# Niema-Lab/AmpliPy

Hardware: AMD Instinct MI355X
Metric: aligned reads/s through trim+pileup+call, 30 kb ref @ 10k x depth (higher is better)
Workload: dtype u8/int32

## Files before the change

### amplipy_amd/build.py

```python
from __future__ import annotations

import os
import shutil
import subprocess

_HERE = os.path.dirname(os.path.abspath(__file__))
CSRC = os.path.join(_HERE, "csrc")
UNITS = ["amplihip.hip", "amp_readpass.hip", "amp_ins.hip", "amp_deflate.hip", "amp_sam.hip", "amp_bgzf.hip", "amp_qc.hip", "amp_strand.hip", "amp_amplicon.hip",
         "amp_codon.hip", "amp_del.hip", "amp_insev.hip", "amp_cooc.hip", "amp_errprof.hip", "amp_hap.hip", "amp_readpos.hip"]
HEADERS = [os.path.join(_HERE, "..", "include", "amplihip.h")] + sorted(os.path.join(CSRC, f) for f in os.listdir(CSRC) if f.endswith(".hpp"))
UNIT_DEPS = {"amplihip.hip": [os.path.join(_HERE, "..", "include", "amplihip.h")] + [os.path.join(CSRC, f) for f in
                              ("amp_ctx.hpp", "amp_read.hpp", "amp_plan.hpp", "amp_hook.hpp", "amp_call.hpp", "amp_ins.hpp", "amp_codec.hpp")],
             "amp_readpass.hip": [os.path.join(_HERE, "..", "include", "amplihip.h")] + [os.path.join(CSRC, f) for f in
                                  ("amp_ctx.hpp", "amp_read.hpp", "amp_plan.hpp", "amp_hook.hpp", "amp_tile.hpp", "amp_bf.hpp", "amp_fast.hpp",
                                   "amp_fast5.hpp", "amp_fast6.hpp", "amp_fast7.hpp", "amp_wave.hpp", "amp_heavy.hpp")],
             "amp_ins.hip": [os.path.join(_HERE, "..", "include", "amplihip.h"), os.path.join(CSRC, "amp_ins.hpp")],
             "amp_deflate.hip": [os.path.join(_HERE, "..", "include", "amplihip.h")],
             "amp_qc.hip": [os.path.join(_HERE, "..", "include", "amplihip.h")] + [os.path.join(CSRC, f) for f in ("amp_hook.hpp", "amp_qc.hpp", "amp_clip.hpp", "amp_strand.hpp", "amp_tally.hpp")],
             "amp_strand.hip": [os.path.join(_HERE, "..", "include", "amplihip.h")] + [os.path.join(CSRC, f) for f in ("amp_hook.hpp", "amp_strand.hpp", "amp_tally.hpp")],
             "amp_amplicon.hip": [os.path.join(_HERE, "..", "include", "amplihip.h")] + [os.path.join(CSRC, f) for f in ("amp_hook.hpp", "amp_strand.hpp", "amp_amplicon.hpp", "amp_tally.hpp")],
             "amp_codon.hip": [os.path.join(_HERE, "..", "include", "amplihip.h")] + [os.path.join(CSRC, f) for f in ("amp_hook.hpp", "amp_strand.hpp", "amp_codon.hpp", "amp_tally.hpp")],
             "amp_del.hip": [os.path.join(_HERE, "..", "include", "amplihip.h")] + [os.path.join(CSRC, f) for f in ("amp_hook.hpp", "amp_strand.hpp", "amp_del.hpp", "amp_keyed.hpp", "amp_tally.hpp")],
             "amp_insev.hip": [os.path.join(_HERE, "..", "include", "amplihip.h")] + [os.path.join(CSRC, f) for f in ("amp_hook.hpp", "amp_strand.hpp", "amp_insev.hpp", "amp_keyed.hpp", "amp_ins.hpp", "amp_readpos.hpp", "amp_tally.hpp")],
             "amp_cooc.hip": [os.path.join(_HERE, "..", "include", "amplihip.h")] + [os.path.join(CSRC, f) for f in ("amp_hook.hpp", "amp_strand.hpp", "amp_cooc.hpp", "amp_tally.hpp")],
             "amp_errprof.hip": [os.path.join(_HERE, "..", "include", "amplihip.h")] + [os.path.join(CSRC, f) for f in ("amp_hook.hpp", "amp_strand.hpp", "amp_errprof.hpp", "amp_tally.hpp")],
             "amp_hap.hip": [os.path.join(_HERE, "..", "include", "amplihip.h")] + [os.path.join(CSRC, f) for f in ("amp_hook.hpp", "amp_strand.hpp", "amp_hap.hpp", "amp_keyed.hpp", "amp_tally.hpp")],
             "amp_readpos.hip": [os.path.join(_HERE, "..", "include", "amplihip.h")] + [os.path.join(CSRC, f) for f in ("amp_hook.hpp", "amp_strand.hpp", "amp_readpos.hpp", "amp_tally.hpp")],
             "amp_sam.hip": [os.path.join(_HERE, "..", "include", "amplihip.h")] + [os.path.join(CSRC, f) for f in
                             ("amp_codec.hpp", "amp_bgzf.hpp", "amp_bamout.hpp", "amp_bamtail.hpp")],
             "amp_bgzf.hip": [os.path.join(_HERE, "..", "include", "amplihip.h")] + [os.path.join(CSRC, f) for f in
                              ("amp_codec.hpp", "amp_bgzf.hpp", "amp_bamout.hpp", "amp_bamtail.hpp", "amp_bamout.hip", "amp_bamtext.hpp", "amp_bamtext.hip")]}
DEPS = [os.path.join(CSRC, u) for u in UNITS] + [os.path.join(CSRC, f) for f in ("amp_bamout.hip", "amp_bamtext.hip")] + HEADERS
OUT = os.path.join(_HERE, "libamplihip.so")
OBJ_DIR = os.path.join(_HERE, "build")
FLAGS = ["-O3", "-std=c++17", "-fPIC", "--offload-arch=gfx950", "-Wall", "-Wno-unused-function"]


def needs_build():
    if not os.path.isfile(OUT):
        return True
    t = os.path.getmtime(OUT)
    return any(os.path.getmtime(d) > t for d in DEPS)


def build(force=False, verbose=False, extra_flags=()):
    if not force and not needs_build():
        return OUT
    hipcc = shutil.which("hipcc") or "/opt/rocm/bin/hipcc"
# ... 38 lines not shown
```

### amplipy_amd/csrc/amp_fast.hpp

```cpp
#pragma once

#include "amp_tile.hpp"
#include "amp_bf.hpp"

namespace amp {

#ifndef AMP_F_LDSPAD
#define AMP_F_LDSPAD 0
#endif
#ifndef AMP_F4_LEAN
#define AMP_F4_LEAN 1
#endif
#ifndef AMP_F4_BF
#define AMP_F4_BF 1
#endif
__device__ __forceinline__ Bf bf_of(const Cig2 &s) { return Bf{s.a, s.m1, s.k, s.m2, s.c, s.kind, s.op, s.punt ? 1u : 0u}; }
__device__ __forceinline__ Cig2 cig2_of(const Bf &b) { return Cig2{b.op, b.a, b.m1, b.k, b.m2, b.c, b.kind, b.punt != 0u}; }
constexpr int F_NP = 10;
constexpr int F_MAXLEN = 152;
constexpr int F_PW = 256;
#ifndef AMP_F_REPS
#define AMP_F_REPS 8
#endif
constexpr int F_REP = AMP_F_REPS;
#ifndef AMP_F_ADD64
#define AMP_F_ADD64 1
#endif
constexpr int F_REPW = F_PW + 1;
#ifndef AMP_F_BW
#define AMP_F_BW 512
#endif
constexpr int F_BW = AMP_F_BW;
constexpr int F_NPL = 4;
constexpr int F_BPL = 6;
constexpr int F_MAXINS = 8;
constexpr int F_MAXDEL = 16;
// ... 221 lines not shown
    atomicMax(&ctr[CTR_STAMP0], f_t[7]); atomicMax(&ctr[CTR_STAMP0 + 1], ~f_t[7]); atomicMax(&ctr[CTR_STAMP0 + 2], ~f_w0); atomicMax(&ctr[CTR_STAMP0 + 3], f_w1); \
    if (f_dbg && wave == 0) { uint32_t *f_o = f_dbg + blockIdx.x * 8; f_o[0] = (uint32_t)f_t[7]; f_o[1] = (uint32_t)f_w0; for (int k = 1; k < 7; ++k) f_o[1 + k] = (uint32_t)(f_t[k] >> 4); } \
    if (f_dbg) { uint32_t *f_o = f_dbg + F_DBG_WAVE0 + (blockIdx.x * F_WAVES + wave) * F_DBG_WAVEWORDS; f_o[0] = (uint32_t)((f_t[1] + f_t[2] + f_t[3] + f_t[4] + f_t[5] + f_t[6]) >> 4); f_o[1] = (uint32_t)(f_epw[0] - f_w0); f_o[2] = (uint32_t)(f_epw[1] - f_epw[0]); f_o[3] = (uint32_t)(f_ep[0] - f_epw[1]); f_o[4] = (uint32_t)(f_ep[1] - f_ep[0]); f_o[5] = (uint32_t)(f_ep[2] - f_ep[1]); } } } while (0)
#else
#define F_DBG_PARAM
#define F_DBG_ARG(x)
#define F_GLOB
#define F_EPIW(k)
#define F_EPI(k)
#define F_STAMP_DECL
#define F_STAMP(k)
#define F_STAMP_VM(k)
#define F_STAMP_OUT
#endif

#define F_ARGS \
    const int32_t *a_pos, int32_t a_min_quality, const uint16_t *a_flag, int32_t a_window, const int32_t *a_tlen, int32_t a_do_trim, \
    const uint32_t *a_lseq, int32_t a_do_count, const uint32_t *a_cig_off32, int32_t a_ref_len, const uint32_t *a_cig, int32_t a_max_primer_len, \
    const uint32_t *a_seq_off8, int32_t reads_per_block, const uint8_t *a_seq, int32_t a_epoch, const uint8_t *a_qual, int32_t pad1, \
    const int32_t *a_min_start, int32_t pad2, const int32_t *a_max_end, int32_t pad3, \
    int32_t *a_new_pos, int32_t pad4, uint32_t *a_new_ncig, int32_t pad5, uint32_t *a_new_cig, int32_t pad6, int32_t *a_o_ref_len, int32_t pad7, \
    uint8_t *a_trim_flags, int32_t pad8, uint8_t *a_status, int32_t pad9, \
    uint32_t *counts, int32_t pad10, amp_ins_event *a_ev, int32_t pad11, unsigned long long *a_ctr, int32_t pad12, uint32_t *a_ins_at, int32_t pad13, \
    uint32_t *glist, int32_t pad14, uint32_t *gcnt, int32_t pad15, \
    int64_t a_n_reads, int32_t pad17, uint64_t read_base, int32_t pad18, long long a_ev_cap
#define F_ARGS_PASS(P, rd, out, eb, rpb) \
    (rd).pos, (P).min_quality, (rd).flag, (P).window, (rd).tlen, (P).do_trim, (rd).lseq, (P).do_count, (rd).cig_off32, (P).ref_len, (rd).cig, \
    (P).max_primer_len, (rd).seq_off8, (rpb), (rd).seq, (int32_t)(P).epoch, (rd).qual, 0, (P).min_start, 0, (P).max_end, 0, (out).new_pos, 0, (out).new_ncig, 0, \
    (out).new_cig, 0, (out).ref_len, 0, (out).trim_flags, 0, (out).status, 0, counts, 0, (eb).ev, 0, (eb).ctr, 0, (eb).ins_at, 0, glist, 0, gcnt, 0, \
    (rd).n_reads, 0, read_base, 0, (eb).cap

enum : uint32_t { KA_MIN_START = 144, KA_MAX_END = 160, KA_NEW_POS = 176, KA_NEW_NCIG = 192, KA_NEW_CIG = 208, KA_O_REF_LEN = 224, KA_TRIM_FLAGS = 240,
                  KA_STATUS = 256, KA_COUNTS = 272, KA_EV = 288, KA_CTR = 304, KA_INS_AT = 320, KA_GLIST = 336, KA_GCNT = 352, KA_N_READS = 368,
                  KA_READ_BASE = 384, KA_EV_CAP = 400 };
static_assert(KA_MAX_END == KA_MIN_START + 16 && KA_NEW_NCIG == KA_NEW_POS + 16 && KA_O_REF_LEN == KA_NEW_CIG + 16 && KA_STATUS == KA_TRIM_FLAGS + 16 &&
              KA_CTR == KA_EV + 16, "karg_late2 reads two neighbours");
template <typename T>
__device__ __forceinline__ T karg_late(uint32_t off) {
    static_assert(sizeof(T) == 8, "the late-loaded arguments are pointers and 64-bit values");
    asm volatile("" : "+s"(off));
    const unsigned long long v = *(const __attribute__((address_space(4))) unsigned long long *)
        ((const __attribute__((address_space(4))) uint8_t *)__builtin_amdgcn_kernarg_segment_ptr() + off);
    return __builtin_bit_cast(T, v);
}
struct KargPair { unsigned long long a, b; };
__device__ __forceinline__ KargPair karg_late2(uint32_t off) {
    typedef unsigned long long amp_u64x4 __attribute__((ext_vector_type(4), aligned(16)));
    asm volatile("" : "+s"(off));
    const amp_u64x4 v = *(const __attribute__((address_space(4))) amp_u64x4 *)
        ((const __attribute__((address_space(4))) uint8_t *)__builtin_amdgcn_kernarg_segment_ptr() + off);
    return KargPair{v.x, v.z};
}
template <typename T>
__device__ __forceinline__ T *karg_late_ptr(uint32_t off) {
    return (T *)karg_late<__attribute__((address_space(1))) T *>(off);
}
template <typename T>
__device__ __forceinline__ T *karg_ptr_of(unsigned long long v) {
    return (T *)__builtin_bit_cast(__attribute__((address_space(1))) T *, v);
}

#if AMP_F_ADD64
#define F_COUNT5(sq, m, d0, lim, wr) count_piece5q(sq, m, d0, lim, wr, (uint32_t)(F_REPW * 4))
#else
#define F_COUNT5(sq, m, d0, lim, wr) count_piece5(sq, m, d0, lim, wr)
#endif
template <int W>
__global__ void __launch_bounds__(F_WAVES * 64, 2)
k_fast(F_ARGS F_DBG_PARAM) {
    const KParams P{a_min_quality, a_window, a_do_trim, a_do_count, a_ref_len, a_max_primer_len, nullptr, nullptr, (uint32_t)a_epoch};
    const amp_dev_reads rd{a_n_reads, a_pos, a_flag, a_tlen, a_lseq, a_cig_off32, a_cig, a_seq_off8, a_seq, a_qual, 0, 0};
    auto late_ctr = [] { return karg_late_ptr<unsigned long long>(KA_CTR); };
    auto late_eb = [] {
        const KargPair ec = karg_late2(KA_EV);
        return EventBuf{karg_ptr_of<amp_ins_event>(ec.a), karg_ptr_of<unsigned long long>(ec.b), karg_late_ptr<uint32_t>(KA_INS_AT), karg_late<long long>(KA_EV_CAP)};
    };
    __shared__ uint4 s_stage[F_WAVES][(F_PAD + F_STAGE + 16) / 16];
    __shared__ __attribute__((aligned(8))) uint32_t s_pwin[F_WAVES][F_REP * F_REPW];
    __shared__ uint32_t s_bwin[F_BPL * F_BW];
    __shared__ uint32_t s_ticket, s_gcur;
#if AMP_F_LDSPAD > 0
    __shared__ uint32_t s_pad[AMP_F_LDSPAD / 4];
    if (P.ref_len == -12345) s_pad[threadIdx.x] = 1;
#endif
// ... 1 lines not shown
    F_STAMP_DECL;
    const int64_t n = rd.n_reads;
    const int64_t rb = (int64_t)blockIdx.x * reads_per_block;
    const int64_t re = rb + reads_per_block < n ? rb + reads_per_block : n;
    lds_u32 *const bwin = (lds_u32 *)s_bwin;
    lds_u32 *const pwin = (lds_u32 *)s_pwin[wave];
    for (int i = tid; i < F_BPL * F_BW; i += F_WAVES * 64) bwin[i] = 0;
    for (int i = lane; i < F_REP * F_REPW; i += 64) pwin[i] = 0;
    if (lane < F_PAD / 4) ((lds_u32 *)s_stage[wave])[lane] = 0x11111111u;
    if (tid == 0) { s_ticket = 0; s_gcur = 0; }
    if (tid == 0 && blockIdx.x == 0) { unsigned long long *const ctr = late_ctr(); ctr[CTR_LONG_N] = 0ull; ctr[CTR_LONG_TICKET] = 0ull; ctr[CTR_GEN_LEFT] = 0ull; }
    int32_t bw_base = rb < n ? rd.pos[rb] : 0;
    bw_base = (bw_base < 16 ? 0 : bw_base - 16) & ~15;
    __syncthreads();

    const int32_t mq = P.min_quality;
    const uint32_t mqc = (uint32_t)(mq > 256 ? 256 : mq);
    const uint32_t thr = mqc * (uint32_t)W;
    const uint32_t mqb = (uint32_t)mq * 0x01010101u;
    const uint32_t G = (uint32_t)P.ref_len;
    const uint32_t n_tb = re > rb ? (uint32_t)((re - rb + 63) / 64) : 0u;
    auto take_ticket = [&]() {
        uint32_t t = 0;
        if (lane == 0) t = __hip_atomic_fetch_add((lds_u32 *)&s_ticket, 1u, __ATOMIC_RELAXED, __HIP_MEMORY_SCOPE_WORKGROUP);
        return (uint32_t)__builtin_amdgcn_readfirstlane((int)t);
    };
    const int64_t wend = re;
    uint32_t n_err = 0;
#ifndef AMP_F_REPSHIFT
#define AMP_F_REPSHIFT 2
#endif
    const uint32_t rep = (F_REP & (F_REP - 1)) ? ((uint32_t)lane >> AMP_F_REPSHIFT) % (uint32_t)F_REP : ((uint32_t)lane >> AMP_F_REPSHIFT) & (uint32_t)(F_REP - 1);
    const uint32_t phi_lane = ((uint32_t)lane >> 1) & 1u ? 8u : 0u;
#if AMP_F_ADD64
    lds_u8 *const wrep = (lds_u8 *)pwin + (rep & (uint32_t)(F_REP / 2 - 1)) * (uint32_t)(2 * F_REPW * 4);
    static_assert((F_REP & 1) == 0 && (F_REPW & 1) == 1, "two arrays per replica, the second one an odd number of words behind the first");
#else
    lds_u8 *const wrep = (lds_u8 *)pwin + rep * (uint32_t)(F_REPW * 4);
#endif
    lds_u8 *const stage = (lds_u8 *)s_stage[wave] + F_PAD;
    int32_t pw_base = 0;
    int pw_tiles = F_FLUSH;
    const unsigned ev_shard = blockIdx.x & (EV_SHARDS - 1);
    unsigned long long ev_base = 0;
    uint32_t ev_left = 0;

    auto fold = [&]() {
        asm volatile("s_waitcnt lgkmcnt(0)" ::: "memory");
        wave_sync();
#pragma unroll 1
        for (int idx = lane; idx < F_PW; idx += 64) {
            uint32_t ag = 0, ct = 0;
#pragma unroll
            for (int r = 0; r < F_REP; ++r) {
                const uint32_t w = pwin[r * F_REPW + idx];
                pwin[r * F_REPW + idx] = 0;
                ag += w & 0x00FF00FFu; ct += (w >> 8) & 0x00FF00FFu;
            }
            if (ag | ct) {
                const int32_t p = pw_base + idx;
                const uint32_t d = (uint32_t)(p - bw_base);
                const uint32_t c4[4] = {ag & 0xFFFFu, ct & 0xFFFFu, ag >> 16, ct >> 16};
#pragma unroll
                for (int c = 0; c < 4; ++c) {
                    if (!c4[c]) continue;
                    if (d < (uint32_t)F_BW) lds_add(bwin + c * F_BW + d, c4[c]);
                    else if ((uint32_t)p < G) { atomicAdd(&karg_late_ptr<uint32_t>(KA_COUNTS)[(size_t)p * AMP_NSYM + c], c4[c]); F_GLOB; }
                }
            }
        }
        wave_sync();
    };
    auto pad_events = [&]() {
        if ((uint32_t)lane < ev_left) {
            const EventBuf eb = late_eb();
            if ((long long)(ev_base + (unsigned)lane) < eb.cap) eb.ev[(size_t)ev_shard * (size_t)eb.cap + ev_base + (unsigned)lane] = amp_ins_event{-1, 0u, 0, 0};
        }
    };

    struct Hdr { int32_t pos, tlen; uint32_t lseq, flag, c0, c1, o8; };
    struct HdrP { int32_t pos; uint32_t lf, c0, o8;
        __device__ uint32_t lseq() const { return lf & 0xFFFFu; }
        __device__ uint32_t nops() const { return (lf >> 19) & 7u; }
        __device__ uint32_t flag() const { return ((lf >> 16) & 1u) | (((lf >> 17) & 1u) << 4); }
        __device__ bool isize_flag() const { return (lf >> 18) & 1u; } };
    auto pack_hdr = [&](const Hdr &h) {
        const uint32_t n = h.c1 - h.c0, at = (uint32_t)(h.tlen < 0 ? -(int64_t)h.tlen : (int64_t)h.tlen);
        const bool isz = ((int64_t)at - P.max_primer_len) > (int64_t)h.lseq;
        return HdrP{h.pos, (h.lseq > 0xFFFFu ? 0xFFFFu : h.lseq) | ((h.flag & 1u) << 16) | (((h.flag >> 4) & 1u) << 17) | ((isz ? 1u : 0u) << 18) | ((n > 7u ? 7u : n) << 19),
                    h.c0, h.o8};
    };
    struct Cg { uint32_t w[5]; };
    struct Geo { uint32_t np, phi, row, Tq; int ntake; bool solo, taken, fastq; };
    struct Tabs { int32_t L, R; };
    struct Bytes { uint4 raws[F_STAGE / 2048]; };
    struct Shape { Cig2 s; bool ok; int32_t refspan; };
    auto load_hdr = [&](int64_t t0) {
        Hdr h{0, 0, 0u, 0u, 0u, 0u, 0u};
        const int64_t i = t0 + lane;
        if (i < wend) {
            h.pos = rd.pos[i]; h.flag = rd.flag[i]; h.tlen = rd.tlen[i]; h.lseq = rd.lseq[i];
            h.c0 = rd.cig_off32[i]; h.c1 = rd.cig_off32[i + 1]; h.o8 = rd.seq_off8[i];
        }
        return h;
    };
    auto load_cig = [&](const HdrP &h) {
        Cg c{{0u, 0u, 0u, 0u, 0u}};
        const uint32_t nops = h.nops();
        if (nops >= 1u && nops <= 5u) {
#pragma unroll
            for (uint32_t k = 0; k < 5u; ++k) c.w[k] = rd.cig[h.c0 + (k < nops ? k : 0u)];
        }
        return c;
    };
    auto geometry = [&](const HdrP &h, int64_t t0, uint32_t &m0) {
        Geo g;
        const bool valid = t0 + lane < wend;
        const uint32_t hl = h.lseq();
        const bool shortq = valid && hl >= 1u && hl <= (uint32_t)F_MAXLEN;
        g.phi = shortq ? phi_lane : 0u;
        g.np = shortq ? (hl + g.phi + 15u) >> 4 : 1u;
        m0 = __builtin_amdgcn_readfirstlane(h.o8);
        g.row = (h.o8 - m0) * 8u;
        const uint32_t nch = (hl + 7u) >> 3;
        const bool fits = valid && h.o8 >= m0 && (h.o8 - m0) <= (uint32_t)(F_STAGE / 8) &&
                          g.row + 8u * nch + (shortq ? 8u : 0u) <= (uint32_t)F_STAGE;
        const unsigned long long fitmask = __ballot(fits);
        g.ntake = fitmask == ~0ull ? 64 : __builtin_ctzll(~fitmask);
        g.solo = g.ntake == 0;
        if (g.solo) g.ntake = 1;
        g.taken = lane < g.ntake && !g.solo;
        g.Tq = g.solo ? 0u : (uint32_t)__builtin_amdgcn_readlane((int)(g.row + 8u * nch), g.ntake - 1);
        g.fastq = g.taken && shortq;
        return g;
    };
    auto shape_of = [&](const HdrP &h, const Cg &c, bool fastq) {
        Shape r;
#if AMP_F4_BF
        bool ok;
        r.s = cig2_of(bf_from_words5((int)h.nops(), c.w[0], c.w[1], c.w[2], c.w[3], c.w[4], fastq ? (int32_t)h.lseq() : 0, F_MAXINS, F_MAXDEL, ok));
        r.ok = ok;
#else
        r.s = Cig2{0u, 0, 0, 0, 0, 0, 0, false};
        const int nops = (int)h.nops();
        r.ok = fastq && nops >= 1 && nops <= 5 && cig2_from_words5(nops, c.w, (int32_t)h.lseq(), r.s);
        if (r.ok && ((r.s.kind == 1 && r.s.k > F_MAXINS) || (r.s.kind == 2 && r.s.k > F_MAXDEL))) r.ok = false;
        if (!r.ok) r.s = Cig2{0u, 0, 0, 0, 0, 0, 0, false};
#endif
        r.refspan = r.ok ? r.s.m1 + r.s.m2 + (r.s.kind == 2 ? r.s.k : 0) : 1;
        return r;
    };
    auto load_tabs = [&](const HdrP &h, const Shape &sh, bool trim) {
        Tabs t{-1, -1};
        const bool in_ref = (uint32_t)h.pos < G && (uint32_t)(h.pos + sh.refspan - 1) < G;
        if (trim && in_ref) {
            const KargPair tabs = karg_late2(KA_MIN_START);
            t.L = karg_ptr_of<const int32_t>(tabs.b)[h.pos]; t.R = karg_ptr_of<const int32_t>(tabs.a)[h.pos + sh.refspan - 1];
        }
        return t;
    };
    auto issue_bytes = [&](const Geo &g, uint32_t m0) {
        Bytes x;
        const uint8_t *qrun = rd.qual + (int64_t)m0 * 8;
        const uint8_t *srun = rd.seq + (int64_t)m0 * 4;
        const uint32_t lastq = g.Tq ? (g.Tq - 1u) & ~15u : 0u, lasts = g.Tq ? ((g.Tq >> 1) - 1u) & ~15u : 0u;
#pragma unroll
        for (int sl = 0; sl < F_STAGE / 1024; ++sl) {
            uint32_t off = (uint32_t)(sl * 1024 + lane * 16);
            off = off < lastq ? off : lastq;
            __builtin_amdgcn_global_load_lds((const __attribute__((address_space(1))) void *)(qrun + off),
                                             (__attribute__((address_space(3))) void *)(stage + sl * 1024), 16, 0, 0);
        }
#pragma unroll
        for (int sl = 0; sl < F_STAGE / 2048; ++sl) {
            uint32_t off = (uint32_t)(sl * 1024 + lane * 16);
            off = off < lasts ? off : lasts;
            const uint32_t *sp = (const uint32_t *)(srun + off);
            x.raws[sl] = make_uint4(sp[0], sp[1], sp[2], sp[3]);
        }
        return x;
    };
    enum : uint32_t { P_STORED = 1u << 24, P_LIST = 1u << 25, P_STATUS_ONLY = 1u << 26 };
    struct Pend { uint32_t i, slot_lo; int32_t pos, reflen; uint32_t meta, cw0, cw1, cw2, cw3, cw4; };
    Pend pend{0u, 0u, 0, 0, 0u, 0u, 0u, 0u, 0u, 0u};
    auto store_pending = [&](const Pend &r) {
#if defined(AMP_DEV) && defined(AMP_ABL)
        if (AMP_ABL & 8) return;
#endif
        const uint32_t ncig = r.meta & 0xFFu;
        if (r.meta & P_STORED) {
            const KargPair o01 = karg_late2(KA_NEW_POS), o23 = karg_late2(KA_NEW_CIG), o45 = karg_late2(KA_TRIM_FLAGS);
            const DevOut out{karg_ptr_of<int32_t>(o01.a), karg_ptr_of<uint32_t>(o01.b), karg_ptr_of<uint32_t>(o23.a),
                             karg_ptr_of<int32_t>(o23.b), karg_ptr_of<uint8_t>(o45.a), karg_ptr_of<uint8_t>(o45.b)};
            uint32_t *home = out.new_cig + ((size_t)r.slot_lo + 3 * (size_t)r.i);
            if (ncig > 0u) home[0] = r.cw0;
            if (ncig > 1u) home[1] = r.cw1;
            if (ncig > 2u) home[2] = r.cw2;
            if (ncig > 3u) home[3] = r.cw3;
            if (ncig > 4u) home[4] = r.cw4;
            if (out.new_pos) out.new_pos[r.i] = r.pos;
            if (out.new_ncig) out.new_ncig[r.i] = ncig;
            if (out.ref_len) out.ref_len[r.i] = r.reflen;
            if (out.trim_flags) out.trim_flags[r.i] = (uint8_t)(r.meta >> 16);
            if (out.status) out.status[r.i] = (uint8_t)(r.meta >> 8);
        }
        const bool has = (r.meta & P_LIST) != 0;
        const unsigned long long m = __ballot(has);
        if (m) {
            uint32_t base = 0;
            if (lane == 0) base = __hip_atomic_fetch_add((lds_u32 *)&s_gcur, (uint32_t)__popcll(m), __ATOMIC_RELAXED, __HIP_MEMORY_SCOPE_WORKGROUP);
            base = (uint32_t)__builtin_amdgcn_readfirstlane((int)base);
            if (has) karg_late_ptr<uint32_t>(KA_GLIST)[(size_t)rb + base + __popcll(m & ((1ull << lane) - 1ull))] = r.i | ((r.meta & P_STATUS_ONLY) ? GL_STATUS_ONLY : 0u);
        }
    };

    uint32_t pw_lim = 0;
    auto count_piece = [&](const uint4 &q, const uint2 &sq, int32_t j0, int32_t qa_, int32_t qb_, int32_t dbase_) -> bool {
        return fast_count_piece(q, sq, j0, qa_, qb_, dbase_, mqb, pw_lim, (uint32_t)(uintptr_t)wrep);
    };

#ifndef AMP_F_STAGGER
#define AMP_F_STAGGER 4000
#endif
    uint32_t tkN = take_ticket(), tkN2 = 0;
    int64_t i0 = rb, i1 = rb + 64 * (int64_t)tkN, i2 = rb;
    const Hdr h_first = load_hdr(i1);
    if (AMP_F_STAGGER > 0) {
        const unsigned long long t_end = __builtin_amdgcn_s_memtime() + (unsigned long long)AMP_F_STAGGER * (unsigned)wave;
        while (__builtin_amdgcn_s_memtime() < t_end) __builtin_amdgcn_s_sleep(8);
    }
    int tile_no = 0; (void)tile_no;
    HdrP hN = pack_hdr(h_first);
    Hdr hN2{0, 0, 0u, 0u, 0u, 0u, 0u};
    Cg cN = load_cig(hN);
    uint32_t m0N = 0;
    Geo gN = geometry(hN, i1, m0N);
    Bytes xN = issue_bytes(gN, m0N);
    tkN2 = take_ticket();
    i2 = rb + 64 * (int64_t)tkN2;
    hN2 = load_hdr(i2);
    while (tkN < n_tb) {
        __builtin_amdgcn_s_waitcnt(0x0F70);
        F_STAMP(1);
#if defined(AMP_DEV) && defined(AMP_ABL)
        if (AMP_ABL & 32) { if (((tile_no++) + (wave >> 2)) & 1) __builtin_amdgcn_s_setprio(1); else __builtin_amdgcn_s_setprio(0); }
#endif
        const HdrP h = hN;
        const Cg cA = cN;
        const Geo g = gN;
        const Bytes xA = xN;
        hN = pack_hdr(hN2);
        i0 = i1; i1 = i2; tkN = tkN2;
        const int64_t i = i0 + lane;
        const int32_t pos = h.pos;
        const uint32_t lseq = h.lseq(), flag = h.flag(), c0 = h.c0, o8 = h.o8;
        const uint32_t np = g.np, phi = g.phi;
        const bool solo = g.solo, taken = g.taken, fastq = g.fastq;
        const Shape shp = shape_of(h, cA, fastq);
        int32_t do_trim_t = P.do_trim, do_count_t = P.do_count;
        asm volatile("" : "+s"(do_trim_t), "+s"(do_count_t));
        const bool trim = shp.ok & (do_trim_t != 0);
        const Tabs tA = load_tabs(h, shp, trim);
        {
            const int32_t first_pos = __builtin_amdgcn_readfirstlane(pos);
            const int32_t want = (first_pos < 16 ? 0 : first_pos - 16) & ~15;
            if (pw_tiles >= F_FLUSH || want < pw_base || want - pw_base >= 64) {
                if (pw_tiles) fold();
                pw_base = want; pw_tiles = 0;
            }
            ++pw_tiles;
        }
        pw_lim = (int64_t)G - pw_base >= (int64_t)F_PW ? (uint32_t)F_PW : (uint32_t)(G > (uint32_t)pw_base ? G - (uint32_t)pw_base : 0u);
        const uint32_t rot = (uint32_t)lane % np;
        const uint8_t *qrow = rd.qual + (int64_t)o8 * 8;
        const uint8_t *srow = rd.seq + (int64_t)o8 * 4;
        const int32_t lrow = fastq ? (int32_t)g.row - (int32_t)phi : 0;
        const lds_u8 *const lq = stage + (fastq ? (int32_t)g.row : 0);
        uint4 q16[F_NP];
        uint2 s8[F_NP];
        wave_sync();
#pragma unroll
        for (int k = 0; k < F_NP; ++k) {
            uint32_t p = (uint32_t)k + rot;
            p = p >= np ? p - np : p;
            p = (uint32_t)k < np ? p : np - 1u;
            const lds_u8 *src = stage + lrow + (int32_t)(p * 16u);
            const amp_u32x2 a = *(const lds_u32x2 *)src, b = *(const lds_u32x2 *)(src + 8);
            q16[k] = make_uint4(a.x, a.y, b.x, b.y);
        }
        Cig2 s = shp.s;
        const bool shaped = shp.ok;
        const bool in_ref = (uint32_t)pos < G && (uint32_t)(pos + shp.refspan - 1) < G;
        const bool rev = (flag & 0x10u) != 0;
        const int32_t q_ins = s.kind ? s.a + s.m1 : 0, q_seg2 = q_ins + (s.kind == 1 ? s.k : 0);
        TrimState ts{pos, 1, 0u, 0};
#if AMP_F4_BF
        {
            ts.err = (trim & !in_ref) ? AMP_RS_INDEX_REF : 0;
            int32_t p2 = pos; uint32_t f2 = 0u;
            s = cig2_of(bf_trim_primers(bf_of(s), p2, f2, flag, h.isize_flag(), (int32_t)lseq, tA.L, tA.R)); ts.pos = p2; ts.flags = f2;
        }
        const bool scan = trim & (ts.err == 0) & !s.punt;
        int32_t lo, qlen;
        bf_quality_window(bf_of(s), (int32_t)lseq, lo, qlen);
        lo = scan ? lo + (int32_t)phi : 0; qlen = scan ? qlen : 0;
#else
        if (trim) {
            if (!in_ref) ts.err = AMP_RS_INDEX_REF;
// ... 13 lines not shown
        wave_sync();
#pragma unroll
        for (int sl = 0; sl < F_STAGE / 2048; ++sl) *(lds_u32x4 *)(stage + sl * 1024 + lane * 16) = amp_u32x4{xA.raws[sl].x, xA.raws[sl].y, xA.raws[sl].z, xA.raws[sl].w};
        wave_sync();
#if AMP_F4_LEAN
        {
            if (lane == 0) *(lds_u32x4 *)(stage + ((g.Tq >> 1) & ~3u)) = amp_u32x4{0x11111111u, 0x11111111u, 0x11111111u, 0x11111111u};
            wave_sync();
            const uint32_t e = fastq ? lseq & 7u : 0u;
            if (e) {
                lds_u32 *w = (lds_u32 *)(stage + (g.row >> 1) + 4u * (lseq >> 3));
                const uint32_t x = *w, xs = ((x & 0x0F0F0F0Fu) << 4) | ((x >> 4) & 0x0F0F0F0Fu);
                const uint32_t keepn = (1u << (4u * e)) - 1u;
                const uint32_t ys = (xs & keepn) | (0x11111111u & ~keepn);
                *w = ((ys & 0x0F0F0F0Fu) << 4) | ((ys >> 4) & 0x0F0F0F0Fu);
            }
            wave_sync();
        }
#endif
#pragma unroll
        for (int k = 0; k < F_NP; ++k) {
            uint32_t p = (uint32_t)k + rot;
            p = p >= np ? p - np : p;
            p = (uint32_t)k < np ? p : np - 1u;
            const lds_u8 *src = stage + (lrow >> 1) + (int32_t)(p * 8u);
            s8[k] = make_uint2(*(const lds_u32 *)src, *(const lds_u32 *)(src + 4));
        }
        const lds_u8 *const lsq = stage + (fastq ? (int32_t)(g.row >> 1) : 0) + (g_b >> 1);
        const uint2 bsq = make_uint2(*(const lds_u32 *)lsq, *(const lds_u32 *)(lsq + 4));
        wave_sync();
        store_pending(pend);
        tkN2 = take_ticket();
        i2 = rb + 64 * (int64_t)tkN2;
        cN = load_cig(hN);
        gN = geometry(hN, i1, m0N);
        xN = issue_bytes(gN, m0N);
        hN2 = load_hdr(i2);
        F_STAMP(2);

        int32_t ffmin = 0x7FFFFFFF, lemax = -1;
#if defined(AMP_DEV) && defined(AMP_ABL)
        if (do_trim_t && !(AMP_ABL & 4)) {
#else
        if (do_trim_t) {
#endif
#pragma unroll
            for (int k = 0; k < F_NP; ++k) {
                uint32_t p = (uint32_t)k + rot;
                p = p >= np ? p - np : p;
                p = (uint32_t)k < np ? p : np;
                const int32_t j0 = (int32_t)(p * 16u);
                uint2 nx = make_uint2(q16[0].x, q16[0].y);
                if (k + 1 < F_NP && (uint32_t)(k + 1) < np) nx = make_uint2(q16[k + 1].x, q16[k + 1].y);
                uint32_t fail = piece_fail_bits<W>(q16[k], nx, thr);
                int32_t blo = lo - j0, bhi = hi - W - j0;
                blo = blo < 0 ? 0 : (blo > 16 ? 16 : blo); bhi = bhi > 15 ? 15 : (bhi < -1 ? -1 : bhi);
                fail &= (0xFFFFu >> (15 - bhi)) & (0xFFFFu << blo);
                const int32_t f1 = j0 + (__builtin_ffs((int)fail) - 1), e1 = j0 + (31 - __builtin_clz(fail)) + W;
                ffmin = fail && f1 < ffmin ? f1 : ffmin;
                lemax = fail && e1 > lemax ? e1 : lemax;
            }
        }

        F_STAMP(3);
        const bool star = fb == 0xFFu;
        int32_t iq = rev ? (lemax >= 0 ? lemax - lo : 0) : (ffmin != 0x7FFFFFFF ? ffmin - lo : qlen);
        const bool tail = scan & (rev ? lemax < 0 : ffmin == 0x7FFFFFFF);
        if (tail) {
            int32_t acc = 0;
            const uint64_t t_lo = (uint64_t)tw0.x | ((uint64_t)tw0.y << 32), t_hi = (uint64_t)tw1.x | ((uint64_t)tw1.y << 32);
            const int32_t kmax = qlen < W - 1 ? qlen : W - 1;
            const int32_t qlo = lo - (int32_t)phi, qhi = hi - (int32_t)phi;
            for (int32_t k = 1; k <= kmax; ++k) {
                const uint32_t o = (uint32_t)((rev ? qlo + k - 1 : qhi - k) - tab);
                acc += (int32_t)(((o < 8u ? t_lo : t_hi) >> ((o & 7u) * 8u)) & 0xFFu);
                if ((int64_t)acc < (int64_t)mq * k) iq = rev ? k : qlen - k;
            }
        }
#if AMP_F4_BF
        { uint32_t f2 = ts.flags; s = cig2_of(bf_trim_quality(bf_of(s), ts.pos, f2, rev, iq, qlen)); ts.flags = f2; }
#else
        if (scan) cig2_trim_quality(ts, rev, iq, qlen, s);
#endif
        const bool stored = shaped & !star & !s.punt;
        const bool general = i < re && !stored;
        const bool emit = stored & (ts.err == 0);
        const bool has0 = emit & (s.a > 0), has1 = emit & (s.m1 > 0), has2 = emit & (s.kind != 0), has3 = has2 & (s.m2 > 0), has4 = emit & (s.c > 0);
        uint32_t cw[5] = {((uint32_t)s.a << 4) | OP_S, ((uint32_t)s.m1 << 4) | s.op, ((uint32_t)s.k << 4) | (s.kind == 1 ? OP_I : OP_D),
                          ((uint32_t)s.m2 << 4) | s.op, ((uint32_t)s.c << 4) | OP_S};
        cw[4] = has4 ? cw[4] : 0u;
        cw[3] = has3 ? cw[3] : cw[4]; cw[4] = has3 ? cw[4] : 0u;
        cw[2] = has2 ? cw[2] : cw[3]; cw[3] = has2 ? cw[3] : cw[4]; cw[4] = has2 ? cw[4] : 0u;
        cw[1] = has1 ? cw[1] : cw[2]; cw[2] = has1 ? cw[2] : cw[3]; cw[3] = has1 ? cw[3] : cw[4]; cw[4] = has1 ? cw[4] : 0u;
        cw[0] = has0 ? cw[0] : cw[1]; cw[1] = has0 ? cw[1] : cw[2]; cw[2] = has0 ? cw[2] : cw[3]; cw[3] = has0 ? cw[3] : cw[4]; cw[4] = has0 ? cw[4] : 0u;
        const uint32_t ncig = (has0 ? 1u : 0u) + (has1 ? 1u : 0u) + (has2 ? 1u : 0u) + (has3 ? 1u : 0u) + (has4 ? 1u : 0u);
        const int32_t reflen = emit ? s.ref_len() : 0;
        n_err += (stored & (ts.err != 0)) ? 1u : 0u;
        const bool counted = stored && !ts.err && do_count_t;
        F_STAMP(4);
        const bool two = counted && s.kind != 0;
// ... 93 lines not shown
#if AMP_F4_LEAN
            const int32_t lim16 = (int32_t)pw_lim - 16;
            if (__ballot(has_b && now)) {
                const uint32_t mB = (has_b & now) ? okB & range_bits16(qa2 - jb, xbe - jb) : 0u;
                redo |= F_COUNT5(bsq, mB, dbase2 + jb, lim16, (uint32_t)(uintptr_t)wrep) << F_NP;
            }
#else
            if (__ballot(has_b && now)) {
                if (has_b && now && count_piece(make_uint4(bq0.x, bq0.y, bq1.x, bq1.y), bsq, jb, qa2, xbe, dbase2)) redo |= 1u << F_NP;
            }
#endif
#pragma unroll
            for (int k = 0; k < F_NP; ++k) {
                uint32_t p = (uint32_t)k + rot;
                p = p >= np ? p - np : p;
                p = (uint32_t)k < np ? p : np;
                const int32_t j0 = (int32_t)(p * 16u);
                const bool second = j0 >= qb1;
#if AMP_F4_LEAN
                redo |= F_COUNT5(s8[k], okm[k] & range_bits16((second ? a2 : a1) - j0, (second ? b2 : b1) - j0), (second ? dbase2 : dbase1) + j0, lim16,
                                 (uint32_t)(uintptr_t)wrep) << k;
#else
                asm volatile("" : "+v"(q16[k].x), "+v"(q16[k].y), "+v"(q16[k].z), "+v"(q16[k].w), "+v"(s8[k].x), "+v"(s8[k].y));
                if (count_piece(q16[k], s8[k], j0, second ? a2 : a1, second ? b2 : b1, second ? dbase2 : dbase1)) redo |= 1u << k;
                __builtin_amdgcn_sched_barrier(0);
#endif
            }
            todo = todo && !now;
        }
        F_STAMP(5);
        bool want_status = bad_extra;
        if (__ballot(redo != 0u)) {
            if (redo) {
                const int32_t a1 = qa1 - (int32_t)phi, b1 = qb1 - (int32_t)phi, a2 = qa2 - (int32_t)phi, b2 = qb2 - (int32_t)phi;
                auto careful = [&](int32_t x0, int32_t x1, int32_t qa_q, int32_t rp0) {
                    for (int32_t q = x0; q < x1; ++q) {
                        if ((int32_t)qrow[q] < mq) continue;
                        const uint32_t sb = srow[q >> 1];
                        const uint32_t col = col_of_code((q & 1) ? (sb & 15u) : (sb >> 4));
                        const int32_t rp = rp0 + (q - qa_q);
                        const uint32_t d = (uint32_t)(rp - bw_base);
                        if (col > 4u || (uint32_t)rp >= G) want_status = true;
                        else if (d < (uint32_t)F_BW && col < (uint32_t)F_NPL) lds_add_nt(bwin + col * F_BW + d, 1u);
                        else atomicAdd(&karg_late_ptr<uint32_t>(KA_COUNTS)[(size_t)rp * AMP_NSYM + col], 1u);
                    }
                };
                for (int k = 0; k < F_NP; ++k) {
                    if (!((redo >> k) & 1u)) continue;
                    uint32_t p = (uint32_t)k + rot;
                    p = p >= np ? p - np : p;
                    const int32_t j0 = (int32_t)(p * 16u) - (int32_t)phi;
                    const bool second = j0 + (int32_t)phi >= qb1;
                    const int32_t sa = second ? a2 : a1, sb_ = second ? b2 : b1;
                    careful(j0 < sa ? sa : j0, j0 + 16 < sb_ ? j0 + 16 : sb_, sa, second ? pos2 : ts.pos);
                }
                if ((redo >> F_NP) & 1u) careful(a2, xbe - (int32_t)phi, a2, pos2);
            }
        }

        {
            uint32_t meta = ncig | ((uint32_t)ts.err << 8) | ((ts.err ? 0u : ts.flags) << 16) | (stored ? P_STORED : 0u);
            if (general) meta |= P_LIST;
            else if (counted && want_status) meta |= P_LIST | P_STATUS_ONLY;
            pend = Pend{(uint32_t)i, c0, ts.pos, reflen, meta, cw[0], cw[1], cw[2], cw[3], cw[4]};
        }
        F_STAMP(6);
// ... 117 lines not shown
```

Before: 10.78 billion.

## Reload kernel arguments lazily via wide kernarg loads, table-based lane rotation, branchless scan

Kernel-argument pointers are reloaded from the kernarg segment with wide scalar loads at each point of use instead of living in registers across the tile loop. This lowers SGPR/VGPR pressure, and the isize bit is now computed once max_primer_len is fetched. lane % np is replaced by a per-lane precomputed packed table when W <= 6. The trim-quality scan's first/last-fail tracking is rewritten with saturating unsigned add/sub to remove branches and compares. The cost is more scalar kernarg loads inside the loop and some extra bit-packing work.

```diff
diff --git a/amplipy_amd/build.py b/amplipy_amd/build.py
--- a/amplipy_amd/build.py
+++ b/amplipy_amd/build.py
@@ -13,7 +13,7 @@
                               ("amp_ctx.hpp", "amp_read.hpp", "amp_plan.hpp", "amp_hook.hpp", "amp_call.hpp", "amp_ins.hpp", "amp_codec.hpp")],
              "amp_readpass.hip": [os.path.join(_HERE, "..", "include", "amplihip.h")] + [os.path.join(CSRC, f) for f in
                                   ("amp_ctx.hpp", "amp_read.hpp", "amp_plan.hpp", "amp_hook.hpp", "amp_tile.hpp", "amp_bf.hpp", "amp_fast.hpp",
-                                   "amp_fast5.hpp", "amp_fast6.hpp", "amp_fast7.hpp", "amp_wave.hpp", "amp_heavy.hpp")],
+                                   "amp_fast5.hpp", "amp_fast6.hpp", "amp_fast7.hpp", "amp_wave.hpp", "amp_heavy.hpp", "amp_scan.hpp")],
              "amp_ins.hip": [os.path.join(_HERE, "..", "include", "amplihip.h"), os.path.join(CSRC, "amp_ins.hpp")],
              "amp_deflate.hip": [os.path.join(_HERE, "..", "include", "amplihip.h")],
              "amp_qc.hip": [os.path.join(_HERE, "..", "include", "amplihip.h")] + [os.path.join(CSRC, f) for f in ("amp_hook.hpp", "amp_qc.hpp", "amp_clip.hpp", "amp_strand.hpp", "amp_tally.hpp")],
diff --git a/amplipy_amd/csrc/amp_fast.hpp b/amplipy_amd/csrc/amp_fast.hpp
--- a/amplipy_amd/csrc/amp_fast.hpp
+++ b/amplipy_amd/csrc/amp_fast.hpp
@@ -2,6 +2,7 @@
 
 #include "amp_tile.hpp"
 #include "amp_bf.hpp"
+#include "amp_scan.hpp"
 
 namespace amp {
 
@@ -289,9 +290,13 @@
 
 enum : uint32_t { KA_MIN_START = 144, KA_MAX_END = 160, KA_NEW_POS = 176, KA_NEW_NCIG = 192, KA_NEW_CIG = 208, KA_O_REF_LEN = 224, KA_TRIM_FLAGS = 240,
                   KA_STATUS = 256, KA_COUNTS = 272, KA_EV = 288, KA_CTR = 304, KA_INS_AT = 320, KA_GLIST = 336, KA_GCNT = 352, KA_N_READS = 368,
-                  KA_READ_BASE = 384, KA_EV_CAP = 400 };
+                  KA_READ_BASE = 384, KA_EV_CAP = 400,
+                  KA_POS = 0, KA_FLAG = 16, KA_DO_TRIM = 40, KA_DO_COUNT = 56, KA_TLEN = 32, KA_LSEQ = 48, KA_CIG_OFF32 = 64, KA_CIG = 80, KA_MAX_PRIMER_LEN = 88, KA_SEQ_OFF8 = 96, KA_SEQ = 112, KA_QUAL = 128 };
 static_assert(KA_MAX_END == KA_MIN_START + 16 && KA_NEW_NCIG == KA_NEW_POS + 16 && KA_O_REF_LEN == KA_NEW_CIG + 16 && KA_STATUS == KA_TRIM_FLAGS + 16 &&
               KA_CTR == KA_EV + 16, "karg_late2 reads two neighbours");
+static_assert(KA_FLAG == KA_POS + 16 && KA_LSEQ == KA_TLEN + 16 && KA_TLEN == KA_POS + 32 && KA_CIG == KA_CIG_OFF32 + 16 && KA_MAX_PRIMER_LEN == KA_CIG + 8 &&
+              KA_SEQ_OFF8 == KA_CIG_OFF32 + 32 && KA_QUAL == KA_SEQ + 16 && KA_MIN_START == KA_QUAL + 16,
+              "the regions of the tile loop: every pointer on the 16-byte pitch, max_primer_len the companion of cig (one x4 load)");
 template <typename T>
 __device__ __forceinline__ T karg_late(uint32_t off) {
     static_assert(sizeof(T) == 8, "the late-loaded arguments are pointers and 64-bit values");
@@ -307,6 +312,26 @@
     const amp_u64x4 v = *(const __attribute__((address_space(4))) amp_u64x4 *)
         ((const __attribute__((address_space(4))) uint8_t *)__builtin_amdgcn_kernarg_segment_ptr() + off);
     return KargPair{v.x, v.z};
+}
+typedef const __attribute__((address_space(4))) uint8_t *karg_base_t;
+__device__ __forceinline__ karg_base_t karg_region() {
+    karg_base_t p = (karg_base_t)__builtin_amdgcn_kernarg_segment_ptr();
+    asm volatile("" : "+s"(p));
+    return p;
+}
+template <int N>
+struct KargWide {
+    uint32_t w[N];
+    __device__ __forceinline__ unsigned long long at(int k) const { return (unsigned long long)w[4 * k] | ((unsigned long long)w[4 * k + 1] << 32); }
+};
+template <int N>
+__device__ __forceinline__ KargWide<N> karg_wide(karg_base_t p, uint32_t off) {
+    typedef uint32_t amp_u32xN __attribute__((ext_vector_type(N), aligned(N >= 4 ? 16 : 4 * N)));
+    const amp_u32xN v = *(const __attribute__((address_space(4))) amp_u32xN *)(p + off);
+    KargWide<N> r;
+#pragma unroll
+    for (int k = 0; k < N; ++k) r.w[k] = v[k];
+    return r;
 }
 template <typename T>
 __device__ __forceinline__ T *karg_late_ptr(uint32_t off) {
@@ -374,6 +399,9 @@
 #endif
     const uint32_t rep = (F_REP & (F_REP - 1)) ? ((uint32_t)lane >> AMP_F_REPSHIFT) % (uint32_t)F_REP : ((uint32_t)lane >> AMP_F_REPSHIFT) & (uint32_t)(F_REP - 1);
     const uint32_t phi_lane = ((uint32_t)lane >> 1) & 1u ? 8u : 0u;
+    constexpr bool rot_by_table = W <= 6;
+    const uint32_t rot_tab = rot_by_table ? fast_rot_table((uint32_t)lane) : 0u;
+    static_assert((F_MAXLEN + 8 + 15) / 16 <= 10, "fast_rot_table holds lane % np for np <= 10");
 #if AMP_F_ADD64
     lds_u8 *const wrep = (lds_u8 *)pwin + (rep & (uint32_t)(F_REP / 2 - 1)) * (uint32_t)(2 * F_REPW * 4);
     static_assert((F_REP & 1) == 0 && (F_REPW & 1) == 1, "two arrays per replica, the second one an odd number of words behind the first");
@@ -426,11 +454,14 @@
         __device__ uint32_t nops() const { return (lf >> 19) & 7u; }
         __device__ uint32_t flag() const { return ((lf >> 16) & 1u) | (((lf >> 17) & 1u) << 4); }
         __device__ bool isize_flag() const { return (lf >> 18) & 1u; } };
-    auto pack_hdr = [&](const Hdr &h) {
+    auto pack_hdr = [&](const Hdr &h, uint32_t &at_out) {
         const uint32_t n = h.c1 - h.c0, at = (uint32_t)(h.tlen < 0 ? -(int64_t)h.tlen : (int64_t)h.tlen);
-        const bool isz = ((int64_t)at - P.max_primer_len) > (int64_t)h.lseq;
-        return HdrP{h.pos, (h.lseq > 0xFFFFu ? 0xFFFFu : h.lseq) | ((h.flag & 1u) << 16) | (((h.flag >> 4) & 1u) << 17) | ((isz ? 1u : 0u) << 18) | ((n > 7u ? 7u : n) << 19),
+        at_out = at;
+        return HdrP{h.pos, (h.lseq > 0xFFFFu ? 0xFFFFu : h.lseq) | ((h.flag & 1u) << 16) | (((h.flag >> 4) & 1u) << 17) | ((n > 7u ? 7u : n) << 19),
                     h.c0, h.o8};
+    };
+    auto isize_bit = [](uint32_t at, uint32_t lseq_raw, int32_t max_primer_len) {
+        return ((int64_t)at - max_primer_len) > (int64_t)lseq_raw ? 1u << 18 : 0u;
     };
     struct Cg { uint32_t w[5]; };
     struct Geo { uint32_t np, phi, row, Tq; int ntake; bool solo, taken, fastq; };
@@ -441,17 +472,29 @@
         Hdr h{0, 0, 0u, 0u, 0u, 0u, 0u};
         const int64_t i = t0 + lane;
         if (i < wend) {
-            h.pos = rd.pos[i]; h.flag = rd.flag[i]; h.tlen = rd.tlen[i]; h.lseq = rd.lseq[i];
-            h.c0 = rd.cig_off32[i]; h.c1 = rd.cig_off32[i + 1]; h.o8 = rd.seq_off8[i];
+            const karg_base_t ka = karg_region();
+            const KargWide<2> b0 = karg_wide<2>(ka, KA_POS), b1 = karg_wide<2>(ka, KA_FLAG), b2 = karg_wide<2>(ka, KA_TLEN), b3 = karg_wide<2>(ka, KA_LSEQ),
+                              b4 = karg_wide<2>(ka, KA_CIG_OFF32), b5 = karg_wide<2>(ka, KA_SEQ_OFF8);
+            const uint32_t *const cig_off32 = karg_ptr_of<const uint32_t>(b4.at(0));
+            h.pos = karg_ptr_of<const int32_t>(b0.at(0))[i]; h.flag = karg_ptr_of<const uint16_t>(b1.at(0))[i];
+            h.tlen = karg_ptr_of<const int32_t>(b2.at(0))[i]; h.lseq = karg_ptr_of<const uint32_t>(b3.at(0))[i];
+            h.c0 = cig_off32[i]; h.c1 = cig_off32[i + 1]; h.o8 = karg_ptr_of<const uint32_t>(b5.at(0))[i];
         }
         return h;
     };
-    auto load_cig = [&](const HdrP &h) {
+    struct ByteBases { const uint32_t *cig; const uint8_t *seq, *qual; int32_t max_primer_len; };
+    auto late_bases = [] {
+        const karg_base_t ka = karg_region();
+        const KargWide<4> c = karg_wide<4>(ka, KA_CIG);
+        const KargWide<2> sb = karg_wide<2>(ka, KA_SEQ), qb = karg_wide<2>(ka, KA_QUAL);
+        return ByteBases{karg_ptr_of<const uint32_t>(c.at(0)), karg_ptr_of<const uint8_t>(sb.at(0)), karg_ptr_of<const uint8_t>(qb.at(0)), (int32_t)c.w[2]};
+    };
+    auto load_cig = [&](const HdrP &h, const uint32_t *cig) {
         Cg c{{0u, 0u, 0u, 0u, 0u}};
         const uint32_t nops = h.nops();
         if (nops >= 1u && nops <= 5u) {
 #pragma unroll
-            for (uint32_t k = 0; k < 5u; ++k) c.w[k] = rd.cig[h.c0 + (k < nops ? k : 0u)];
+            for (uint32_t k = 0; k < 5u; ++k) c.w[k] = cig[h.c0 + (k < nops ? k : 0u)];
         }
         return c;
     };
@@ -492,26 +535,26 @@
         r.refspan = r.ok ? r.s.m1 + r.s.m2 + (r.s.kind == 2 ? r.s.k : 0) : 1;
         return r;
     };
-    auto load_tabs = [&](const HdrP &h, const Shape &sh, bool trim) {
+    auto load_tabs = [&](const HdrP &h, const Shape &sh, bool trim, const int32_t *tab_l, const int32_t *tab_r) {
         Tabs t{-1, -1};
         const bool in_ref = (uint32_t)h.pos < G && (uint32_t)(h.pos + sh.refspan - 1) < G;
         if (trim && in_ref) {
-            const KargPair tabs = karg_late2(KA_MIN_START);
-            t.L = karg_ptr_of<const int32_t>(tabs.b)[h.pos]; t.R = karg_ptr_of<const int32_t>(tabs.a)[h.pos + sh.refspan - 1];
+            t.L = tab_l[h.pos]; t.R = tab_r[h.pos + sh.refspan - 1];
         }
         return t;
     };
-    auto issue_bytes = [&](const Geo &g, uint32_t m0) {
+    auto issue_bytes = [&](const Geo &g, uint32_t m0, const ByteBases &bb) {
         Bytes x;
-        const uint8_t *qrun = rd.qual + (int64_t)m0 * 8;
-        const uint8_t *srun = rd.seq + (int64_t)m0 * 4;
+        const uint8_t *qrun = bb.qual + (int64_t)m0 * 8;
+        const uint8_t *srun = bb.seq + (int64_t)m0 * 4;
         const uint32_t lastq = g.Tq ? (g.Tq - 1u) & ~15u : 0u, lasts = g.Tq ? ((g.Tq >> 1) - 1u) & ~15u : 0u;
+        lds_u8 *const stage_u = (lds_u8 *)(uintptr_t)(uint32_t)__builtin_amdgcn_readfirstlane((int)(uint32_t)(uintptr_t)stage);
 #pragma unroll
         for (int sl = 0; sl < F_STAGE / 1024; ++sl) {
             uint32_t off = (uint32_t)(sl * 1024 + lane * 16);
             off = off < lastq ? off : lastq;
             __builtin_amdgcn_global_load_lds((const __attribute__((address_space(1))) void *)(qrun + off),
-                                             (__attribute__((address_space(3))) void *)(stage + sl * 1024), 16, 0, 0);
+                                             (__attribute__((address_space(3))) void *)(stage_u + sl * 1024), 16, 0, 0);
         }
 #pragma unroll
         for (int sl = 0; sl < F_STAGE / 2048; ++sl) {
@@ -531,9 +574,11 @@
 #endif
         const uint32_t ncig = r.meta & 0xFFu;
         if (r.meta & P_STORED) {
-            const KargPair o01 = karg_late2(KA_NEW_POS), o23 = karg_late2(KA_NEW_CIG), o45 = karg_late2(KA_TRIM_FLAGS);
-            const DevOut out{karg_ptr_of<int32_t>(o01.a), karg_ptr_of<uint32_t>(o01.b), karg_ptr_of<uint32_t>(o23.a),
-                             karg_ptr_of<int32_t>(o23.b), karg_ptr_of<uint8_t>(o45.a), karg_ptr_of<uint8_t>(o45.b)};
+            const karg_base_t ka = karg_region();
+            const KargWide<2> o0 = karg_wide<2>(ka, KA_NEW_POS), o1 = karg_wide<2>(ka, KA_NEW_NCIG), o2 = karg_wide<2>(ka, KA_NEW_CIG),
+                              o3 = karg_wide<2>(ka, KA_O_REF_LEN), o4 = karg_wide<2>(ka, KA_TRIM_FLAGS), o5 = karg_wide<2>(ka, KA_STATUS);
+            const DevOut out{karg_ptr_of<int32_t>(o0.at(0)), karg_ptr_of<uint32_t>(o1.at(0)), karg_ptr_of<uint32_t>(o2.at(0)),
+                             karg_ptr_of<int32_t>(o3.at(0)), karg_ptr_of<uint8_t>(o4.at(0)), karg_ptr_of<uint8_t>(o5.at(0))};
             uint32_t *home = out.new_cig + ((size_t)r.slot_lo + 3 * (size_t)r.i);
             if (ncig > 0u) home[0] = r.cw0;
             if (ncig > 1u) home[1] = r.cw1;
@@ -572,17 +617,25 @@
         while (__builtin_amdgcn_s_memtime() < t_end) __builtin_amdgcn_s_sleep(8);
     }
     int tile_no = 0; (void)tile_no;
-    HdrP hN = pack_hdr(h_first);
+    uint32_t at_first = 0;
+    HdrP hN = pack_hdr(h_first, at_first);
     Hdr hN2{0, 0, 0u, 0u, 0u, 0u, 0u};
-    Cg cN = load_cig(hN);
+    const ByteBases bb_first = late_bases();
+    hN.lf |= isize_bit(at_first, h_first.lseq, bb_first.max_primer_len);
+    Cg cN = load_cig(hN, bb_first.cig);
     uint32_t m0N = 0;
     Geo gN = geometry(hN, i1, m0N);
-    Bytes xN = issue_bytes(gN, m0N);
+    Bytes xN = issue_bytes(gN, m0N, bb_first);
     tkN2 = take_ticket();
     i2 = rb + 64 * (int64_t)tkN2;
     hN2 = load_hdr(i2);
     while (tkN < n_tb) {
+        const karg_base_t ka_top = karg_region();
+        const int32_t do_trim_k = (int32_t)karg_wide<1>(ka_top, KA_DO_TRIM).w[0], do_count_k = (int32_t)karg_wide<1>(ka_top, KA_DO_COUNT).w[0];
+        const KargWide<2> tab_lw = karg_wide<2>(ka_top, KA_MAX_END), tab_rw = karg_wide<2>(ka_top, KA_MIN_START);
+        unsigned long long tab_l = tab_lw.at(0), tab_r = tab_rw.at(0);
         __builtin_amdgcn_s_waitcnt(0x0F70);
+        asm volatile("" : "+s"(tab_l), "+s"(tab_r));
         F_STAMP(1);
 #if defined(AMP_DEV) && defined(AMP_ABL)
         if (AMP_ABL & 32) { if (((tile_no++) + (wave >> 2)) & 1) __builtin_amdgcn_s_setprio(1); else __builtin_amdgcn_s_setprio(0); }
@@ -591,7 +644,8 @@
         const Cg cA = cN;
         const Geo g = gN;
         const Bytes xA = xN;
-        hN = pack_hdr(hN2);
+        uint32_t atN = 0; const uint32_t lseqN_raw = hN2.lseq;
+        hN = pack_hdr(hN2, atN);
         i0 = i1; i1 = i2; tkN = tkN2;
         const int64_t i = i0 + lane;
         const int32_t pos = h.pos;
@@ -599,10 +653,10 @@
         const uint32_t np = g.np, phi = g.phi;
         const bool solo = g.solo, taken = g.taken, fastq = g.fastq;
         const Shape shp = shape_of(h, cA, fastq);
-        int32_t do_trim_t = P.do_trim, do_count_t = P.do_count;
+        int32_t do_trim_t = do_trim_k, do_count_t = do_count_k;
         asm volatile("" : "+s"(do_trim_t), "+s"(do_count_t));
         const bool trim = shp.ok & (do_trim_t != 0);
-        const Tabs tA = load_tabs(h, shp, trim);
+        const Tabs tA = load_tabs(h, shp, trim, karg_ptr_of<const int32_t>(tab_l), karg_ptr_of<const int32_t>(tab_r));
         {
             const int32_t first_pos = __builtin_amdgcn_readfirstlane(pos);
             const int32_t want = (first_pos < 16 ? 0 : first_pos - 16) & ~15;
@@ -613,9 +667,7 @@
             ++pw_tiles;
         }
         pw_lim = (int64_t)G - pw_base >= (int64_t)F_PW ? (uint32_t)F_PW : (uint32_t)(G > (uint32_t)pw_base ? G - (uint32_t)pw_base : 0u);
-        const uint32_t rot = (uint32_t)lane % np;
-        const uint8_t *qrow = rd.qual + (int64_t)o8 * 8;
-        const uint8_t *srow = rd.seq + (int64_t)o8 * 4;
+        const uint32_t rot = rot_by_table ? fast_rot(rot_tab, np) : (uint32_t)lane % np;
         const int32_t lrow = fastq ? (int32_t)g.row - (int32_t)phi : 0;
         const lds_u8 *const lq = stage + (fastq ? (int32_t)g.row : 0);
         uint4 q16[F_NP];
@@ -695,13 +747,15 @@
         store_pending(pend);
         tkN2 = take_ticket();
         i2 = rb + 64 * (int64_t)tkN2;
-        cN = load_cig(hN);
+        const ByteBases bbN = late_bases();
+        hN.lf |= isize_bit(atN, lseqN_raw, bbN.max_primer_len);
+        cN = load_cig(hN, bbN.cig);
         gN = geometry(hN, i1, m0N);
-        xN = issue_bytes(gN, m0N);
+        xN = issue_bytes(gN, m0N, bbN);
         hN2 = load_hdr(i2);
         F_STAMP(2);
 
-        int32_t ffmin = 0x7FFFFFFF, lemax = -1;
+        uint32_t ffmin = SCAN_NO_START, lemax = SCAN_NO_END;
 #if defined(AMP_DEV) && defined(AMP_ABL)
         if (do_trim_t && !(AMP_ABL & 4)) {
 #else
@@ -716,19 +770,15 @@
                 uint2 nx = make_uint2(q16[0].x, q16[0].y);
                 if (k + 1 < F_NP && (uint32_t)(k + 1) < np) nx = make_uint2(q16[k + 1].x, q16[k + 1].y);
                 uint32_t fail = piece_fail_bits<W>(q16[k], nx, thr);
-                int32_t blo = lo - j0, bhi = hi - W - j0;
-                blo = blo < 0 ? 0 : (blo > 16 ? 16 : blo); bhi = bhi > 15 ? 15 : (bhi < -1 ? -1 : bhi);
-                fail &= (0xFFFFu >> (15 - bhi)) & (0xFFFFu << blo);
-                const int32_t f1 = j0 + (__builtin_ffs((int)fail) - 1), e1 = j0 + (31 - __builtin_clz(fail)) + W;
-                ffmin = fail && f1 < ffmin ? f1 : ffmin;
-                lemax = fail && e1 > lemax ? e1 : lemax;
+                fail &= scan_start_bits(lo, hi, W, j0);
+                scan_piece(fail, (uint32_t)j0, p * 16u + (uint32_t)(W + 31), ffmin, lemax);
             }
         }
 
         F_STAMP(3);
         const bool star = fb == 0xFFu;
-        int32_t iq = rev ? (lemax >= 0 ? lemax - lo : 0) : (ffmin != 0x7FFFFFFF ? ffmin - lo : qlen);
-        const bool tail = scan & (rev ? lemax < 0 : ffmin == 0x7FFFFFFF);
+        int32_t iq = rev ? (lemax != SCAN_NO_END ? (int32_t)lemax - lo : 0) : (ffmin != SCAN_NO_START ? (int32_t)ffmin - lo : qlen);
+        const bool tail = scan & (rev ? lemax == SCAN_NO_END : ffmin == SCAN_NO_START);
         if (tail) {
             int32_t acc = 0;
             const uint64_t t_lo = (uint64_t)tw0.x | ((uint64_t)tw0.y << 32), t_hi = (uint64_t)tw1.x | ((uint64_t)tw1.y << 32);
@@ -888,6 +938,9 @@
         bool want_status = bad_extra;
         if (__ballot(redo != 0u)) {
             if (redo) {
+                const KargPair sqb = karg_late2(KA_SEQ);
+                const uint8_t *qrow = karg_ptr_of<const uint8_t>(sqb.b) + (int64_t)o8 * 8;
+                const uint8_t *srow = karg_ptr_of<const uint8_t>(sqb.a) + (int64_t)o8 * 4;
                 const int32_t a1 = qa1 - (int32_t)phi, b1 = qb1 - (int32_t)phi, a2 = qa2 - (int32_t)phi, b2 = qb2 - (int32_t)phi;
                 auto careful = [&](int32_t x0, int32_t x1, int32_t qa_q, int32_t rp0) {
                     for (int32_t q = x0; q < x1; ++q) {
diff --git a/amplipy_amd/csrc/amp_scan.hpp b/amplipy_amd/csrc/amp_scan.hpp
--- /dev/null
+++ b/amplipy_amd/csrc/amp_scan.hpp
@@ -0,0 +1,36 @@
+#pragma once
+
+#include "amp_read.hpp"
+
+namespace amp {
+
+AMP_HD uint32_t fast_rot_table(uint32_t lane) {
+    constexpr uint32_t M[10] = {512u, 256u, 171u, 128u, 103u, 86u, 74u, 64u, 57u, 52u};
+    uint32_t t = 0;
+#pragma unroll
+    for (uint32_t n = 1; n <= 10u; ++n) {
+        const uint32_t q = (lane * M[n - 1u]) >> 9;
+        t |= (lane - q * n) << (n <= 8u ? 3u * (n - 1u) : 24u + 4u * (n - 9u));
+    }
+    return t;
+}
+AMP_HD uint32_t fast_rot(uint32_t table, uint32_t np) {
+    const uint32_t off = 3u * np - 3u + (np > 9u ? 1u : 0u), width = np > 8u ? 4u : 3u;
+    return (table >> off) & ((1u << width) - 1u);
+}
+
+constexpr uint32_t SCAN_NO_START = 0xFFFFFFFFu, SCAN_NO_END = 0u;
+AMP_HD uint32_t scan_umin(uint32_t a, uint32_t b) { return a < b ? a : b; }
+AMP_HD uint32_t scan_umax(uint32_t a, uint32_t b) { return a > b ? a : b; }
+AMP_HD void scan_piece(uint32_t fail, uint32_t j0, uint32_t endw, uint32_t &first_start, uint32_t &last_end) {
+    const uint32_t lowest = fail ? (uint32_t)__builtin_ctz(fail) : 0xFFFFFFFFu, zeros = fail ? (uint32_t)__builtin_clz(fail) : 0xFFFFFFFFu;
+    first_start = scan_umin(first_start, __builtin_elementwise_add_sat(lowest, j0));
+    last_end = scan_umax(last_end, __builtin_elementwise_sub_sat(endw, zeros));
+}
+AMP_HD uint32_t scan_start_bits(int32_t lo, int32_t hi, int32_t W, int32_t j0) {
+    int32_t blo = lo - j0, bhi = hi - W - j0;
+    blo = blo < 0 ? 0 : (blo > 16 ? 16 : blo); bhi = bhi > 15 ? 15 : (bhi < -1 ? -1 : bhi);
+    return (0xFFFFu >> (15 - bhi)) & (0xFFFFu << blo);
+}
+
+}
```

After: 10.83 billion, median of 2. No clear change (+0.4%).
